# samxuxiang/BrepGen

Hardware: AMD Instinct MI355X
Metric: denoising-steps/sec (whole node), DeepCAD face-LDM, batch=512 (higher is better)
Workload: dtype bf16

## Files before the change

### brepgen_amd/csrc/qkv_attn.hip

```cpp
#include "gemm16.h"
#include <math.h>

namespace bg {

constexpr int QA_BUF = 57344, QA_AHALF = 16384, QA_WOFF = 32768, QA_RING = 2 * QA_BUF;
constexpr int QA_LDS = 163840;
constexpr int QA_AUX = QA_RING, QA_BIAS = QA_LDS - QA_AUX - 2048, QA_CSUM = QA_BIAS + 1024;
constexpr int QA_QIMG = QA_BUF, QA_KIMG = QA_QIMG + 32768, QA_VIMG = QA_KIMG + 32768;

constexpr int QA_MB = QA_AUX + QA_BIAS - 1024;
static_assert(QA_VIMG + 32768 <= QA_MB && QA_VIMG + 32768 <= QA_AUX + QA_BIAS, "the V image ends below the key bias / bias / column sums");

struct QkvAttnArgs {
    const void* a;
    const void* w;
    const float* bias;
    const float* colsum;
    const float* stats_in;
    void* out;
    void* dbg;
    const uint8_t* key_pad;
    int B, N, M;
    float ln_eps;
    const int* m_dev = nullptr;
    const int* slot_desc = nullptr;
    int pin = 0;
};

typedef __attribute__((ext_vector_type(4))) short qa_v4s;

__device__ __forceinline__ int qa_opaque(int x) {
    asm volatile("" : "+v"(x));
    return x;
}

template <bool F16, int S, bool MASK, bool DBG = false, bool PAIR = false>
__global__ __launch_bounds__(512) void qkv_attn_kernel(QkvAttnArgs g) {
    using E = Elem<F16>;
    using T = typename E::T;
    using V8 = typename E::V8;
    using V4 = typename E::V4;
    constexpr int SPT = 256 / S;
    constexpr int WPS = S / 32;
    constexpr int LD = BG_D_MODEL;
    __shared__ __attribute__((aligned(16))) unsigned char lds[QA_LDS];

    const int wave = __builtin_amdgcn_readfirstlane(threadIdx.x >> 6);
    const int wm = wave >> 1, wn = (wave ^ (wave >> 2)) & 1;
    const int late = wave >> 2;
    static_assert(!PAIR || (S == 64 && !MASK), "slot-packed batches: 64-row slots, dead keys come from the slot descriptors");
    const int Mv = PAIR ? *g.m_dev : 0;
    const int n_groups = PAIR ? (Mv + 255) >> 8 : (g.B + SPT - 1) / SPT;
    const int T_all = n_groups * BG_N_HEAD;
    const int G = gridDim.x;
    int L = xcd_remap(blockIdx.x, G);
    const bool pin = g.pin != 0;
    const int pin_q = (blockIdx.x & 7) >> 1, pin_h0 = (blockIdx.x & 1) * 6, pin_step = G >> 3;
    auto tile_of = [&](int l, int& tg, int& th) -> bool {
        if (pin) { tg = 4 * (l / 6) + pin_q; th = pin_h0 + l % 6; return tg < n_groups; }
        tg = l / BG_N_HEAD; th = l % BG_N_HEAD;
        return l < T_all;
    };
    if (pin) L = blockIdx.x >> 3;
    {
        int tg, th;
        if (!tile_of(L, tg, th)) return;
    }

    const unsigned char* Ab = reinterpret_cast<const unsigned char*>(g.a);
    const unsigned char* Wb = reinterpret_cast<const unsigned char*>(g.w);
    constexpr unsigned lda_b = LD * 2u, ldw_b = LD * 2u;
    const unsigned lds0 = __builtin_amdgcn_readfirstlane((unsigned)(size_t)(__attribute__((address_space(3))) void*)lds);
    const unsigned aux_lds = lds0 + QA_AUX;
    const unsigned char* aux = lds + QA_AUX;

    auto dma = [&](unsigned dst, const unsigned char* src, unsigned voff) {
        unsigned keep;
        asm volatile("s_mov_b32 %0, m0\n\ts_mov_b32 m0, %3\n\ts_nop 0\n\tglobal_load_lds_dwordx4 %1, %2\n\ts_mov_b32 m0, %0"
                     : "=&s"(keep) : "v"(voff), "s"(src), "s"(dst) : "memory");
    };

    auto bar = [&]() {
        asm volatile("" ::: "memory");
        __builtin_amdgcn_sched_barrier(0);
        __builtin_amdgcn_s_barrier();
        __builtin_amdgcn_sched_barrier(0);
        asm volatile("" ::: "memory");
    };
    auto lds_done_bar = [&]() {
        asm volatile("s_waitcnt lgkmcnt(0)" ::: "memory");
        bar();
    };

    unsigned ha[2][2], hw;
    auto piece_row = [&](int ln, int r) { return (wave + 8 * r) * 8 + (ln >> 3); };
    auto piece_chunk = [&](int ln, int r) { return (unsigned)(((ln & 7) ^ ((piece_row(ln, r) >> 1) & 7)) * 16); };
    auto slot_row = [&](int grp, int tile_row) {
        if (PAIR) {
            const int row = grp * 256 + tile_row;
            return row < Mv ? row : Mv - 1;
        }
        int smp = grp * SPT + tile_row / S;
        smp = smp < g.B ? smp : g.B - 1;
        int tok = tile_row % S;
        tok = tok < g.N ? tok : g.N - 1;
        return smp * g.N + tok;
    };
    auto a_offsets = [&](int grp) {
        const int ln = qa_opaque(threadIdx.x & 63);
#pragma unroll
        for (int hh = 0; hh < 2; ++hh)
#pragma unroll
            for (int r = 0; r < 2; ++r)
                ha[hh][r] = (unsigned)slot_row(grp, hh * 128 + piece_row(ln, r)) * lda_b + piece_chunk(ln, r);
    };
    {
        const int ln = threadIdx.x & 63;
        hw = (unsigned)piece_row(ln, 0) * ldw_b + piece_chunk(ln, 0);
    }
    auto stage_a = [&](int buf, const unsigned char* src) {
#pragma unroll
        for (int hh = 0; hh < 2; ++hh)
#pragma unroll
            for (int r = 0; r < 2; ++r)
                dma(lds0 + (unsigned)(buf * QA_BUF + hh * QA_AHALF + (wave + 8 * r) * 1024), src, ha[hh][r]);
    };
    auto stage_w = [&](int buf, const unsigned char* src) {
#pragma unroll
        for (int c3 = 0; c3 < 3; ++c3)
            dma(lds0 + (unsigned)(buf * QA_BUF + QA_WOFF + (wave + 8 * c3) * 1024), src + (size_t)c3 * LD * ldw_b, hw);
    };
    auto stage_stats = [&](int grp) {
        const int ln = qa_opaque(threadIdx.x & 63);
        const int gh = wave >> 2;
        int row = slot_row(grp, gh * 128 + 2 * ln);
        row = (row & 1) ? row - 1 : row;
        const unsigned char* sb = reinterpret_cast<const unsigned char*>(g.stats_in);
#pragma unroll
        for (int r = 0; r < 3; ++r) {
            const int part = (wave & 3) * 3 + r;
            dma(aux_lds + (unsigned)(gh * 12288 + part * 1024), sb + (size_t)part * (size_t)g.M * 8, (unsigned)(row >> 1) * 16u);
        }
    };
    auto stage_cols = [&](int head) {
        const int ln = qa_opaque(threadIdx.x & 63);
        int c3 = ln >> 4;
        c3 = c3 < 3 ? c3 : 2;
        const unsigned voff = (unsigned)(c3 * LD + (ln & 15) * 4) * 4u;
        if (wave == 0) dma(aux_lds + QA_BIAS, reinterpret_cast<const unsigned char*>(g.bias + head * 64), voff);
        if (wave == 1) dma(aux_lds + QA_CSUM, reinterpret_cast<const unsigned char*>(g.colsum + head * 64), voff);
    };

    unsigned a_rd, b_rd, xk[4];
    {
        const int ln = threadIdx.x & 63, l31 = ln & 31, hq = ln >> 5, sw = (l31 >> 1) & 7;
        a_rd = (unsigned)(wm * 64 + l31) * 128u;
        b_rd = (unsigned)QA_WOFF + (unsigned)(wn * 96 + l31) * 128u;
#pragma unroll
        for (int ks = 0; ks < 4; ++ks) xk[ks] = (unsigned)(((ks * 2 + hq) ^ sw) << 4);
    }
    f32x16 acc[2][3];
    V8 fa[2][4], fb[3][4];
    auto read_a = [&](const unsigned char* st) {
#pragma unroll
        for (int i = 0; i < 2; ++i)
#pragma unroll
            for (int ks = 0; ks < 4; ++ks) fa[i][ks] = *reinterpret_cast<const V8*>(st + a_rd + i * 4096 + xk[ks]);
    };
    auto read_b = [&](const unsigned char* st, int j) {
#pragma unroll
        for (int ks = 0; ks < 4; ++ks) fb[j][ks] = *reinterpret_cast<const V8*>(st + b_rd + j * 4096 + xk[ks]);
    };
    auto segment = [&](int j) {
        asm volatile("s_waitcnt lgkmcnt(0)" ::: "memory");
        __builtin_amdgcn_sched_barrier(0);
        __builtin_amdgcn_s_setprio(1);
#pragma unroll
        for (int ks = 0; ks < 4; ++ks)
#pragma unroll
            for (int i = 0; i < 2; ++i) acc[i][j] = E::mfma(fb[j][ks], fa[i][ks], acc[i][j]);
        __builtin_amdgcn_s_setprio(0);
        __builtin_amdgcn_sched_barrier(0);
    };

    constexpr int KT = LD / G_BK;
    const unsigned char* b0 = lds;
    const unsigned char* b1 = lds + QA_BUF;

    int grp, head;
    tile_of(L, grp, head);
    float2 cf[2];
    auto fold_sums = [&](int i) {
        const int l31 = qa_opaque(threadIdx.x & 31);
        const unsigned char* sg = aux + (wm >> 1) * 12288;
        const int rg = (wm & 1) * 64 + i * 32 + l31;
        float ps[16], pq[16];
#pragma unroll
        for (int pp = 0; pp < 16; ++pp) {
            const float2 v = pp < FOLD_PARTS ? reinterpret_cast<const float2*>(sg + pp * 1024)[rg] : make_float2(0.f, 0.f);
            ps[pp] = v.x; pq[pp] = v.y;
        }
        cf[i] = make_float2(tree16(ps), tree16(pq));
        asm volatile("" : "+v"(cf[i].x), "+v"(cf[i].y) :: "memory");
        __builtin_amdgcn_sched_barrier(0);
    };
    auto fold_coeffs = [&](int i) {
        cf[i] = ln_fold_coeffs(cf[i].x, cf[i].y, LD, g.ln_eps);
        asm volatile("" : "+v"(cf[i].x), "+v"(cf[i].y) :: "memory");
        __builtin_amdgcn_sched_barrier(0);
    };

    a_offsets(grp);
    stage_stats(grp); stage_cols(head);
    stage_a(0, Ab); stage_w(0, Wb + (size_t)head * 64 * ldw_b); stage_a(1, Ab + 2 * G_BK);
    wait_vmcnt<4>();
    bar();
    for (;;) {
        if (late) bar();
        const unsigned char* w_cur = Wb + (size_t)head * 64 * ldw_b;
        const int Ln = L + (pin ? pin_step : G);
        int grp_n, head_n;
        const bool has_next = tile_of(Ln, grp_n, head_n);
        const unsigned char* w_nxt = Wb + (size_t)head_n * 64 * ldw_b;
#pragma unroll
        for (int i = 0; i < 2; ++i)
#pragma unroll
            for (int j = 0; j < 3; ++j)
#pragma unroll
                for (int r = 0; r < 16; ++r) acc[i][j][r] = 0.f;

        auto iteration = [&](const unsigned char* w1, bool more, const unsigned char* a2, const unsigned char* w2, bool more3,
                             const unsigned char* a3, int fold) {
            read_b(b0, 0); __builtin_amdgcn_sched_barrier(0); read_a(b0);
            stage_w(1, w1);
            bar(); segment(0); bar();
            read_b(b0, 1); read_b(b0, 2);
            bar(); segment(1); bar();
            if (more) { stage_a(0, a2); wait_vmcnt<4>(); } else { wait_vmcnt<0>(); }
            if (fold >= 0) fold_sums(fold);
            bar(); segment(2); bar();
            read_b(b1, 0); __builtin_amdgcn_sched_barrier(0); read_a(b1);
            if (more) stage_w(0, w2);
            bar(); segment(0); bar();
            read_b(b1, 1); read_b(b1, 2);
            bar(); segment(1); bar();
            if (more3) { stage_a(1, a3); wait_vmcnt<4>(); } else if (more) { wait_vmcnt<0>(); }
            if (fold >= 0) fold_coeffs(fold);
            bar(); segment(2); bar();
        };
        for (int t = 0; t + 2 < KT; t += 2) {
            const unsigned kb = (unsigned)t * (2 * G_BK);
            iteration(w_cur + kb + 2 * G_BK, true, Ab + kb + 4 * G_BK, w_cur + kb + 4 * G_BK, true, Ab + kb + 6 * G_BK,
                      t == KT - 6 ? 0 : (t == KT - 4 ? 1 : -1));
        }
        if (has_next) a_offsets(grp_n);
        iteration(w_cur + (unsigned)(KT - 1) * (2 * G_BK), has_next, Ab, w_nxt, false, Ab, -1);
        if (!late) bar();

        const int ln = qa_opaque(threadIdx.x & 63), l31 = ln & 31, hq = ln >> 5;
        T* dbg = reinterpret_cast<T*>(g.dbg);
        int pair_na = 64, pair_nb = 0;
        if (PAIR) {
            const int gslot = grp * 4 + wm;
            if (gslot * 64 < Mv) { pair_na = g.slot_desc[2 * gslot]; pair_nb = g.slot_desc[2 * gslot + 1]; }
            pair_na = __builtin_amdgcn_readfirstlane(pair_na);
            pair_nb = __builtin_amdgcn_readfirstlane(pair_nb);
        }
        float key_bias = 0.f;
        if (MASK && threadIdx.x < 256) {
            const int smp = grp * SPT + (int)threadIdx.x / S, key = (int)threadIdx.x % S;
            const bool inside = smp < g.B && key < g.N;
            const uint8_t pad = inside ? g.key_pad[(size_t)smp * g.N + key] : (uint8_t)1;
            key_bias = pad ? -INFINITY : 0.f;
        }
#pragma unroll
        for (int j = 0; j < 3; ++j) {
            const int tc0 = wn * 96 + j * 32;
            const int c3 = tc0 >> 6, d0 = tc0 & 63;
#pragma unroll
            for (int q = 0; q < 4; ++q) {
                const int d = d0 + 8 * q + 4 * hq;
                const float4 bz = *reinterpret_cast<const float4*>(aux + QA_BIAS + (unsigned)(c3 * 64 + d) * 4u);
                const float4 cs = *reinterpret_cast<const float4*>(aux + QA_CSUM + (unsigned)(c3 * 64 + d) * 4u);
                const float b4[4] = {bz.x, bz.y, bz.z, bz.w}, c4[4] = {cs.x, cs.y, cs.z, cs.w};
#pragma unroll
                for (int i = 0; i < 2; ++i) {
                    float v[4];
#pragma unroll
                    for (int e = 0; e < 4; ++e) v[e] = ln_fold_apply(acc[i][j][4 * q + e], cf[i].x, cf[i].y, c4[e], b4[e]);
                    if (F16) asm volatile("" : "+v"(v[0]), "+v"(v[1]), "+v"(v[2]), "+v"(v[3]));
                    union { V4 v; uint2 u; T t[4]; } pk;
                    pk.v = E::pack4(v[0], v[1], v[2], v[3]);
                    const int R = wm * 64 + i * 32 + l31;
                    *reinterpret_cast<uint2*>(lds + QA_QIMG + c3 * 32768 + R * 128 + ((((d >> 3) ^ ((R >> 1) & 7))) << 4) + (d & 7) * 2) = pk.u;
                    if (DBG) {
                        const int smp = grp * SPT + R / S, tok = R % S;
                        if (PAIR ? grp * 256 + R < Mv : (smp < g.B && tok < g.N))
                            *reinterpret_cast<uint2*>(dbg + (size_t)(PAIR ? grp * 256 + R : smp * g.N + tok) * (3 * LD) + c3 * LD + head * 64 + d) = pk.u;
                    }
                }
            }
        }
        if (MASK && threadIdx.x < 256) reinterpret_cast<float*>(lds + QA_MB)[threadIdx.x] = key_bias;
        lds_done_bar();

        if (has_next) stage_cols(head_n);

        {
            const int wq = wm * 2 + wn;
            const int slot = wq / WPS, qb = wq % WPS;
            const int smp = grp * SPT + slot;
            if (PAIR ? (grp * 256 + slot * 64 < Mv) : (smp < g.B)) {
                const int h = hq;
                const unsigned char* qimg = lds + QA_QIMG + (slot * S + qb * 32) * 128;
                const unsigned char* ktile = lds + QA_KIMG + slot * S * 128;
                const unsigned char* vimg = lds + QA_VIMG + slot * S * 128;
                const int gi = ln & 15, gg = ln >> 4;
                const int v_key0 = 4 * (gg >> 1) + (gi >> 2);
                int v_c16[2], v_b8;
                v_b8 = ((gi & 3) * 4 & 7) * 2;
#pragma unroll
                for (int dt = 0; dt < 2; ++dt) v_c16[dt] = (dt * 32 + (gg & 1) * 16 + (gi & 3) * 4) >> 3;
                const int sw = (l31 >> 1) & 7;
                V8 qf[4];
#pragma unroll
                for (int ks = 0; ks < 4; ++ks) qf[ks] = *reinterpret_cast<const V8*>(qimg + l31 * 128 + (((ks * 2 + h) ^ sw) << 4));
                f32x16 o[2];
#pragma unroll
                for (int dt = 0; dt < 2; ++dt)
#pragma unroll
                    for (int r = 0; r < 16; ++r) o[dt][r] = 0.f;
                float m_run = -INFINITY, l_run = 0.f;
                const int tq = qb * 32 + l31;
                const bool in_b = PAIR && tq >= pair_na && tq < pair_na + pair_nb;
                bool first = true;
#pragma unroll
                for (int si = 0; si < (PAIR ? 2 : 1); ++si) {
                    const int cnt = PAIR ? (si == 0 ? pair_na : pair_nb) : g.N;
                    const int row0 = (PAIR && si == 1) ? pair_na : 0;
                    const bool member = !PAIR || (in_b == (si == 1));
                    if (PAIR && __ballot(member) == 0ull) continue;
#pragma unroll
                    for (int sub = 0; sub < WPS; ++sub) {
                        if (sub * 32 >= cnt) break;
                        f32x16 s;
#pragma unroll
                        for (int r = 0; r < 16; ++r) s[r] = 0.f;
                        int kr = row0 + sub * 32 + l31;
                        if (PAIR) kr = kr < 63 ? kr : 63;
                        const int ksw = PAIR ? (kr >> 1) & 7 : sw;
#pragma unroll
                        for (int ks = 0; ks < 4; ++ks) {
                            const V8 kf = *reinterpret_cast<const V8*>(ktile + kr * 128 + (((ks * 2 + h) ^ ksw) << 4));
                            s = E::mfma(kf, qf[ks], s);
                        }
                        if (MASK) {
                            const float* mb = reinterpret_cast<const float*>(lds + QA_MB) + slot * S + sub * 32 + 4 * h;
#pragma unroll
                            for (int g4 = 0; g4 < 4; ++g4) {
                                const float4 mbv = *reinterpret_cast<const float4*>(mb + 8 * g4);
                                s[4 * g4 + 0] += mbv.x; s[4 * g4 + 1] += mbv.y; s[4 * g4 + 2] += mbv.z; s[4 * g4 + 3] += mbv.w;
                            }
                        } else if (PAIR) {
                            const int thr = member ? cnt - sub * 32 - 4 * h : -64;
#pragma unroll
                            for (int r = 0; r < 16; ++r) s[r] += ((r & 3) + 8 * (r >> 2)) >= thr ? -INFINITY : 0.f;
                        } else if (sub * 32 + 32 > g.N) {
                            const int thr = g.N - sub * 32 - 4 * h;
#pragma unroll
                            for (int r = 0; r < 16; ++r) s[r] += ((r & 3) + 8 * (r >> 2)) >= thr ? -INFINITY : 0.f;
                        }
                        float mloc = -INFINITY;
#pragma unroll
                        for (int g4 = 0; g4 < 4; ++g4)
                            mloc = fmaxf(mloc, fmaxf(fmaxf(s[4 * g4 + 0], s[4 * g4 + 1]), fmaxf(s[4 * g4 + 2], s[4 * g4 + 3])));
                        mloc = fmaxf(mloc, __shfl_xor(mloc, 32, 64));
                        const float m_new = fmaxf(m_run, mloc);
                        const float m_use = (m_new == -INFINITY) ? 0.f : m_new;
                        float psum = 0.f;
#pragma unroll
                        for (int r = 0; r < 16; ++r) {
                            s[r] = __expf(s[r] - m_use);
                            psum += s[r];
                        }
                        if (first) {
                            l_run = psum;
                        } else {
                            const float alpha = __expf(m_run - m_use);
                            l_run = l_run * alpha + psum;
#pragma unroll
                            for (int dt = 0; dt < 2; ++dt)
#pragma unroll
                                for (int r = 0; r < 16; ++r) o[dt][r] *= alpha;
                        }
                        first = false;
                        m_run = m_new;
#pragma unroll
                        for (int sl = 0; sl < 2; ++sl) {
                            V8 pb;
#pragma unroll
                            for (int e = 0; e < 8; ++e) pb[e] = (T)s[8 * sl + e];
                            int r_lo = row0 + sub * 32 + 16 * sl + v_key0, r_hi = r_lo + 8;
                            if (PAIR) { r_lo = r_lo < 63 ? r_lo : 63; r_hi = r_hi < 63 ? r_hi : 63; }
#pragma unroll
                            for (int dt = 0; dt < 2; ++dt) {
                                const unsigned char* pl = vimg + r_lo * 128 + ((v_c16[dt] ^ ((r_lo >> 1) & 7)) << 4) + v_b8;
                                const unsigned char* ph = vimg + r_hi * 128 + ((v_c16[dt] ^ ((r_hi >> 1) & 7)) << 4) + v_b8;
                                union { qa_v4s s4[2]; V8 v; } vau;
                                vau.s4[0] = __builtin_amdgcn_ds_read_tr16_b64_v4i16((__attribute__((address_space(3))) qa_v4s*)pl);
                                vau.s4[1] = __builtin_amdgcn_ds_read_tr16_b64_v4i16((__attribute__((address_space(3))) qa_v4s*)ph);
                                const V8 va = vau.v;
                                o[dt] = E::mfma(va, pb, o[dt]);
                            }
                        }
                    }
                }
                const float l_tot = l_run + __shfl_xor(l_run, 32, 64);
                const float inv = l_tot > 0.f ? 1.0f / l_tot : 0.f;
                if (PAIR || tq < g.N) {
                    T* op = reinterpret_cast<T*>(g.out) + (size_t)(PAIR ? grp * 256 + slot * 64 + tq : smp * g.N + tq) * LD + head * 64;
#pragma unroll
                    for (int dt = 0; dt < 2; ++dt)
#pragma unroll
                        for (int k2 = 0; k2 < 2; ++k2) {
                            union { V4 v; unsigned u[2]; } q0, q1;
                            q0.v[0] = cvt16<T>(o[dt][8 * k2 + 0] * inv); q0.v[1] = cvt16<T>(o[dt][8 * k2 + 1] * inv);
                            q0.v[2] = cvt16<T>(o[dt][8 * k2 + 2] * inv); q0.v[3] = cvt16<T>(o[dt][8 * k2 + 3] * inv);
                            q1.v[0] = cvt16<T>(o[dt][8 * k2 + 4] * inv); q1.v[1] = cvt16<T>(o[dt][8 * k2 + 5] * inv);
                            q1.v[2] = cvt16<T>(o[dt][8 * k2 + 6] * inv); q1.v[3] = cvt16<T>(o[dt][8 * k2 + 7] * inv);
                            const auto w0 = __builtin_amdgcn_permlane32_swap(q0.u[0], q1.u[0], false, false);
                            const auto w1 = __builtin_amdgcn_permlane32_swap(q0.u[1], q1.u[1], false, false);
                            const uint4 st16 = make_uint4(w0[0], w1[0], w0[1], w1[1]);
                            *reinterpret_cast<uint4*>(op + dt * 32 + 16 * k2 + 8 * h) = st16;
                        }
                }
            }
        }
        if (!has_next) break;
        lds_done_bar();
        L = Ln; grp = grp_n; head = head_n;
        stage_a(1, Ab + 2 * G_BK);
        stage_stats(grp);
    }
}

bool qkv_attn_eligible(int B, int N, int dtype, const void* stats_in, const void* colsum, const void* bias) {
    return (dtype == BG_BF16 || dtype == BG_F16) && B > 0 && N >= 2 && N <= 64 && (N & 1) == 0 && stats_in && colsum && bias &&
           (((size_t)stats_in) & 15) == 0 && (size_t)B * N * BG_D_MODEL * 2 < 0xffffffffull;
}

bool qkv_attn_worthwhile(int B, int N) {
    const int spt = N <= 32 ? 8 : 4;
    const int tiles = (B + spt - 1) / spt * BG_N_HEAD;
    return tiles <= 256 || tiles >= 352;
}

static int qkv_attn_pinned_walk(int tiles, int grid) {
    const int t = g_tune[TUNE_QKV_WALK];
    if (t == 1 || (grid & 7) != 0) return 0;
    return (t == 2 || tiles >= 512) ? 1 : 0;
}

int qkv_attention_launch(const QkvAttnArgs& g, int dtype, hipStream_t s) {
    const int S = g.N <= 32 ? 32 : 64, spt = 256 / S;
    const int tiles = (g.B + spt - 1) / spt * BG_N_HEAD;
    if (tiles <= 0) return 0;
    const double rows = (double)g.B * g.N;
    ProfScope prof(PK_QKV_ATTN, 2.0 * rows * BG_D_MODEL * 3 * BG_D_MODEL + 4.0 * BG_N_HEAD * (double)g.B * g.N * g.N * BG_D_HEAD,
                   rows * (2.0 * BG_D_MODEL * 2 + FOLD_PARTS * 8.0) + 2.0 * 3 * BG_D_MODEL * BG_D_MODEL + 2 * 4.0 * 3 * BG_D_MODEL, s);
    const int grid = tiles < 256 ? tiles : 256;
    const bool f16 = dtype == BG_F16;
    QkvAttnArgs ge = g;
    ge.pin = qkv_attn_pinned_walk(tiles, grid);
#define QA_LAUNCH(F, SS, MK, D) hipLaunchKernelGGL((qkv_attn_kernel<F, SS, MK, D>), dim3(grid), dim3(512), 0, s, ge)
#define QA_PICK(MK, D)                                                                                     \
    do {                                                                                                   \
        if (S == 64) { if (f16) QA_LAUNCH(true, 64, MK, D); else QA_LAUNCH(false, 64, MK, D); }           \
        else { if (f16) QA_LAUNCH(true, 32, MK, D); else QA_LAUNCH(false, 32, MK, D); }                   \
    } while (0)
    if (g.dbg) {
        if (g.key_pad) QA_PICK(true, true); else QA_PICK(false, true);
    } else {
        if (g.key_pad) QA_PICK(true, false); else QA_PICK(false, false);
    }
#undef QA_PICK
#undef QA_LAUNCH
    return launch_status("qkv_attn");
}

int qkv_attention_paired(const void* x_hi, const void* w_qkv, const float* bias, const float* colsum, const float* stats_in, void* out,
                         void* qkv_dbg, const int* m_dev, const int* slot_desc, int slot_bound, int m_stats, int dtype, float ln_eps,
                         hipStream_t s, double rows_hint, double pairs_hint) {
    if (slot_bound <= 0) return 0;
    QkvAttnArgs g{x_hi, w_qkv, bias, colsum, stats_in, out, qkv_dbg, nullptr, slot_bound, 64, m_stats, ln_eps};
    g.m_dev = m_dev;
    g.slot_desc = slot_desc;
    const int tiles = (slot_bound + 3) / 4 * BG_N_HEAD;
    g.pin = qkv_attn_pinned_walk(tiles, tiles < 256 ? tiles : 256);
    const double rows = rows_hint > 0 ? rows_hint : 64.0 * slot_bound;
    const double pairs = pairs_hint > 0 ? pairs_hint : 64.0 * rows;
    ProfScope prof(PK_QKV_ATTN, 2.0 * rows * BG_D_MODEL * 3 * BG_D_MODEL + 4.0 * BG_N_HEAD * pairs * BG_D_HEAD,
                   rows * (2.0 * BG_D_MODEL * 2 + FOLD_PARTS * 8.0) + 2.0 * 3 * BG_D_MODEL * BG_D_MODEL + 2 * 4.0 * 3 * BG_D_MODEL, s);
    const int grid = tiles < 256 ? tiles : 256;
    if (dtype == BG_F16) {
        if (qkv_dbg) hipLaunchKernelGGL((qkv_attn_kernel<true, 64, false, true, true>), dim3(grid), dim3(512), 0, s, g);
        else hipLaunchKernelGGL((qkv_attn_kernel<true, 64, false, false, true>), dim3(grid), dim3(512), 0, s, g);
    } else {
        if (qkv_dbg) hipLaunchKernelGGL((qkv_attn_kernel<false, 64, false, true, true>), dim3(grid), dim3(512), 0, s, g);
        else hipLaunchKernelGGL((qkv_attn_kernel<false, 64, false, false, true>), dim3(grid), dim3(512), 0, s, g);
    }
    return launch_status("qkv_attn_paired");
}

int qkv_attention(const void* x_hi, const void* w_qkv, const float* bias, const float* colsum, const float* stats_in, void* out,
                  const uint8_t* key_pad, int B, int N, int dtype, float ln_eps, hipStream_t s) {
    const QkvAttnArgs g{x_hi, w_qkv, bias, colsum, stats_in, out, nullptr, key_pad, B, N, B * N, ln_eps};
    return qkv_attention_launch(g, dtype, s);
}

}

extern "C" int bg_qkv_attn_fwd(const void* x_hi, const void* w_qkv, const float* bias, const float* colsum, const float* stats_in,
                               const uint8_t* key_pad, void* out, void* qkv_dbg, int B, int N, int dtype, float ln_eps,
                               bg_stream_t stream) {
    BG_REQUIRE(x_hi && w_qkv && out && B >= 0 && N >= 0, BG_E_ARG, "bg_qkv_attn_fwd: null pointer or negative size");
    BG_REQUIRE(bg::qkv_attn_eligible(B, N, dtype, stats_in, colsum, bias), BG_E_SHAPE,
               "bg_qkv_attn_fwd: needs 16-bit operands, an even N in [2, 64], LayerNorm-fold statistics / column sums / bias (16-byte aligned)");
    BG_REQUIRE(((uintptr_t)x_hi & 15) == 0 && ((uintptr_t)w_qkv & 15) == 0 && ((uintptr_t)out & 15) == 0 &&
               ((uintptr_t)bias & 15) == 0 && ((uintptr_t)colsum & 15) == 0, BG_E_ALIGN, "bg_qkv_attn_fwd: 16-byte alignment");
    bg::QkvAttnArgs g{x_hi, w_qkv, bias, colsum, stats_in, out, qkv_dbg, key_pad, B, N, B * N, ln_eps};
    return bg::qkv_attention_launch(g, dtype, (hipStream_t)stream);
}

extern "C" int bg_qkv_attn_paired_fwd(const void* x_hi, const void* w_qkv, const float* bias, const float* colsum, const float* stats_in,
                                      void* out, void* qkv_dbg, const int* m_dev, const int* slot_desc, int slot_bound, int m_stats,
                                      int dtype, float ln_eps, bg_stream_t stream) {
    BG_REQUIRE(x_hi && w_qkv && out && m_dev && slot_desc && slot_bound > 0 && m_stats >= 64 * slot_bound, BG_E_ARG,
               "bg_qkv_attn_paired_fwd: null pointer, or a statistics stride below 64 rows per slot");
    BG_REQUIRE((dtype == BG_BF16 || dtype == BG_F16) && stats_in && colsum && bias && (m_stats & 1) == 0, BG_E_SHAPE,
               "bg_qkv_attn_paired_fwd: 16-bit operands with LayerNorm-fold statistics / column sums / bias");
    BG_REQUIRE(((uintptr_t)x_hi & 15) == 0 && ((uintptr_t)w_qkv & 15) == 0 && ((uintptr_t)out & 15) == 0 && ((uintptr_t)bias & 15) == 0 &&
               ((uintptr_t)colsum & 15) == 0 && ((uintptr_t)stats_in & 15) == 0, BG_E_ALIGN, "bg_qkv_attn_paired_fwd: 16-byte alignment");
    BG_REQUIRE((size_t)64 * slot_bound * BG_D_MODEL * 2 < 0xffffffffull, BG_E_SHAPE, "bg_qkv_attn_paired_fwd: more than 43 690 slots");
    return bg::qkv_attention_paired(x_hi, w_qkv, bias, colsum, stats_in, out, qkv_dbg, m_dev, slot_desc, slot_bound, m_stats, dtype, ln_eps,
                                    (hipStream_t)stream, 0.0, 0.0);
}
```

Before: 370.5.

## Replace block barrier with pairwise wave flags and batch attention LDS loads

In the unmasked path, the block-wide barrier between writing the Q/K/V images and the attention phase becomes a pairwise handshake through LDS flags, so each wave waits only on its partner wave. The attention inner loop now loads all K and V fragments for a sample up front before issuing the MFMAs. The loop is templated on sub-tile count, and the cross-half shuffles use permlane32_swap instead of __shfl_xor. Bias and column-sum loads are hoisted into registers, and stage_cols moves after the end-of-tile barrier. The risks are higher register pressure and the correctness of the flag protocol, which assumes only the partner wave's image rows are read. Optional timestamp probes are added behind a macro.

```diff
diff --git a/brepgen_amd/csrc/qkv_attn.hip b/brepgen_amd/csrc/qkv_attn.hip
--- a/brepgen_amd/csrc/qkv_attn.hip
+++ b/brepgen_amd/csrc/qkv_attn.hip
@@ -1,5 +1,6 @@
 #include "gemm16.h"
 #include <math.h>
+#include <type_traits>
 
 namespace bg {
 
@@ -10,6 +11,8 @@
 
 constexpr int QA_MB = QA_AUX + QA_BIAS - 1024;
 static_assert(QA_VIMG + 32768 <= QA_MB && QA_VIMG + 32768 <= QA_AUX + QA_BIAS, "the V image ends below the key bias / bias / column sums");
+constexpr int QA_FLAG = QA_VIMG + 32768;
+static_assert(QA_FLAG + 32 <= QA_MB, "the image flags end below the key bias");
 
 struct QkvAttnArgs {
     const void* a;
@@ -25,7 +28,21 @@
     const int* m_dev = nullptr;
     const int* slot_desc = nullptr;
     int pin = 0;
+#ifdef QA_STAMPS
+    long long* stamps = nullptr;
+#endif
 };
+
+#ifdef QA_STAMPS
+constexpr int QA_STAMP_TILES = 16;
+#define QA_STAMP(k)                                                                                                              \
+    do {                                                                                                                         \
+        if (g.stamps && blockIdx.x == 0 && (threadIdx.x & 255) == 0 && n_tile < QA_STAMP_TILES)                                 \
+            g.stamps[((threadIdx.x >> 8) * QA_STAMP_TILES + n_tile) * 8 + (k)] = (long long)__builtin_amdgcn_s_memtime();      \
+    } while (0)
+#else
+#define QA_STAMP(k) do {} while (0)
+#endif
 
 typedef __attribute__((ext_vector_type(4))) short qa_v4s;
 
@@ -213,10 +230,17 @@
     a_offsets(grp);
     stage_stats(grp); stage_cols(head);
     stage_a(0, Ab); stage_w(0, Wb + (size_t)head * 64 * ldw_b); stage_a(1, Ab + 2 * G_BK);
+    volatile __attribute__((address_space(3))) int* img_flag = (volatile __attribute__((address_space(3))) int*)(lds + QA_FLAG);
+    if ((threadIdx.x & 63) == 0) img_flag[wave] = 0;
+    int img_seq = 0;
     wait_vmcnt<4>();
     bar();
+#ifdef QA_STAMPS
+    int n_tile = 0;
+#endif
     for (;;) {
         if (late) bar();
+        QA_STAMP(0);
         const unsigned char* w_cur = Wb + (size_t)head * 64 * ldw_b;
         const int Ln = L + (pin ? pin_step : G);
         int grp_n, head_n;
@@ -256,6 +280,7 @@
         if (has_next) a_offsets(grp_n);
         iteration(w_cur + (unsigned)(KT - 1) * (2 * G_BK), has_next, Ab, w_nxt, false, Ab, -1);
         if (!late) bar();
+        QA_STAMP(1);
 
         const int ln = qa_opaque(threadIdx.x & 63), l31 = ln & 31, hq = ln >> 5;
         T* dbg = reinterpret_cast<T*>(g.dbg);
@@ -273,6 +298,15 @@
             const uint8_t pad = inside ? g.key_pad[(size_t)smp * g.N + key] : (uint8_t)1;
             key_bias = pad ? -INFINITY : 0.f;
         }
+        float4 bzq[3][4], csq[3][4];
+#pragma unroll
+        for (int j = 0; j < 3; ++j)
+#pragma unroll
+            for (int q = 0; q < 4; ++q) {
+                const unsigned col = (unsigned)(wn * 96 + j * 32 + 8 * q + 4 * hq);
+                bzq[j][q] = *reinterpret_cast<const float4*>(aux + QA_BIAS + col * 4u);
+                csq[j][q] = *reinterpret_cast<const float4*>(aux + QA_CSUM + col * 4u);
+            }
 #pragma unroll
         for (int j = 0; j < 3; ++j) {
             const int tc0 = wn * 96 + j * 32;
@@ -280,8 +314,7 @@
 #pragma unroll
             for (int q = 0; q < 4; ++q) {
                 const int d = d0 + 8 * q + 4 * hq;
-                const float4 bz = *reinterpret_cast<const float4*>(aux + QA_BIAS + (unsigned)(c3 * 64 + d) * 4u);
-                const float4 cs = *reinterpret_cast<const float4*>(aux + QA_CSUM + (unsigned)(c3 * 64 + d) * 4u);
+                const float4 bz = bzq[j][q], cs = csq[j][q];
                 const float b4[4] = {bz.x, bz.y, bz.z, bz.w}, c4[4] = {cs.x, cs.y, cs.z, cs.w};
 #pragma unroll
                 for (int i = 0; i < 2; ++i) {
@@ -301,10 +334,19 @@
                 }
             }
         }
-        if (MASK && threadIdx.x < 256) reinterpret_cast<float*>(lds + QA_MB)[threadIdx.x] = key_bias;
-        lds_done_bar();
-
-        if (has_next) stage_cols(head_n);
+        QA_STAMP(2);
+        if (MASK) {
+            if (threadIdx.x < 256) reinterpret_cast<float*>(lds + QA_MB)[threadIdx.x] = key_bias;
+            lds_done_bar();
+        } else {
+            ++img_seq;
+            asm volatile("s_waitcnt lgkmcnt(0)" ::: "memory");
+            if (ln == 0) img_flag[wave] = img_seq;
+            while (__builtin_amdgcn_readfirstlane(img_flag[wave ^ 1]) != img_seq) __builtin_amdgcn_s_sleep(1);
+            asm volatile("" ::: "memory");
+            __builtin_amdgcn_sched_barrier(0);
+        }
+        QA_STAMP(3);
 
         {
             const int wq = wm * 2 + wn;
@@ -334,26 +376,49 @@
                 const int tq = qb * 32 + l31;
                 const bool in_b = PAIR && tq >= pair_na && tq < pair_na + pair_nb;
                 bool first = true;
-#pragma unroll
-                for (int si = 0; si < (PAIR ? 2 : 1); ++si) {
-                    const int cnt = PAIR ? (si == 0 ? pair_na : pair_nb) : g.N;
-                    const int row0 = (PAIR && si == 1) ? pair_na : 0;
-                    const bool member = !PAIR || (in_b == (si == 1));
-                    if (PAIR && __ballot(member) == 0ull) continue;
-#pragma unroll
-                    for (int sub = 0; sub < WPS; ++sub) {
-                        if (sub * 32 >= cnt) break;
-                        f32x16 s;
-#pragma unroll
-                        for (int r = 0; r < 16; ++r) s[r] = 0.f;
+                auto other_half = [&](float x) {
+                    const auto p2 = __builtin_amdgcn_permlane32_swap(__float_as_uint(x), __float_as_uint(x), false, false);
+                    return __uint_as_float(h ? p2[0] : p2[1]);
+                };
+                auto sample = [&](auto ns_tag, int cnt, int row0, bool member) {
+                    constexpr int NS = decltype(ns_tag)::value;
+                    V8 kf[NS][4], va[NS][2][2];
+#pragma unroll
+                    for (int sub = 0; sub < NS; ++sub) {
                         int kr = row0 + sub * 32 + l31;
                         if (PAIR) kr = kr < 63 ? kr : 63;
                         const int ksw = PAIR ? (kr >> 1) & 7 : sw;
 #pragma unroll
-                        for (int ks = 0; ks < 4; ++ks) {
-                            const V8 kf = *reinterpret_cast<const V8*>(ktile + kr * 128 + (((ks * 2 + h) ^ ksw) << 4));
-                            s = E::mfma(kf, qf[ks], s);
+                        for (int ks = 0; ks < 4; ++ks) kf[sub][ks] = *reinterpret_cast<const V8*>(ktile + kr * 128 + (((ks * 2 + h) ^ ksw) << 4));
+                    }
+#pragma unroll
+                    for (int sub = 0; sub < NS; ++sub)
+#pragma unroll
+                        for (int sl = 0; sl < 2; ++sl) {
+                            int r_lo = row0 + sub * 32 + 16 * sl + v_key0, r_hi = r_lo + 8;
+                            if (PAIR) { r_lo = r_lo < 63 ? r_lo : 63; r_hi = r_hi < 63 ? r_hi : 63; }
+#pragma unroll
+                            for (int dt = 0; dt < 2; ++dt) {
+                                const unsigned char* pl = vimg + r_lo * 128 + ((v_c16[dt] ^ ((r_lo >> 1) & 7)) << 4) + v_b8;
+                                const unsigned char* ph = vimg + r_hi * 128 + ((v_c16[dt] ^ ((r_hi >> 1) & 7)) << 4) + v_b8;
+                                union { qa_v4s s4[2]; V8 v; } vau;
+                                vau.s4[0] = __builtin_amdgcn_ds_read_tr16_b64_v4i16((__attribute__((address_space(3))) qa_v4s*)pl);
+                                vau.s4[1] = __builtin_amdgcn_ds_read_tr16_b64_v4i16((__attribute__((address_space(3))) qa_v4s*)ph);
+                                va[sub][sl][dt] = vau.v;
+                            }
                         }
+                    f32x16 sc[NS];
+#pragma unroll
+                    for (int sub = 0; sub < NS; ++sub)
+#pragma unroll
+                        for (int r = 0; r < 16; ++r) sc[sub][r] = 0.f;
+#pragma unroll
+                    for (int ks = 0; ks < 4; ++ks)
+#pragma unroll
+                        for (int sub = 0; sub < NS; ++sub) sc[sub] = E::mfma(kf[sub][ks], qf[ks], sc[sub]);
+#pragma unroll
+                    for (int sub = 0; sub < NS; ++sub) {
+                        f32x16& s = sc[sub];
                         if (MASK) {
                             const float* mb = reinterpret_cast<const float*>(lds + QA_MB) + slot * S + sub * 32 + 4 * h;
 #pragma unroll
@@ -374,7 +439,7 @@
 #pragma unroll
                         for (int g4 = 0; g4 < 4; ++g4)
                             mloc = fmaxf(mloc, fmaxf(fmaxf(s[4 * g4 + 0], s[4 * g4 + 1]), fmaxf(s[4 * g4 + 2], s[4 * g4 + 3])));
-                        mloc = fmaxf(mloc, __shfl_xor(mloc, 32, 64));
+                        mloc = fmaxf(mloc, other_half(mloc));
                         const float m_new = fmaxf(m_run, mloc);
                         const float m_use = (m_new == -INFINITY) ? 0.f : m_new;
                         float psum = 0.f;
@@ -400,22 +465,21 @@
                             V8 pb;
 #pragma unroll
                             for (int e = 0; e < 8; ++e) pb[e] = (T)s[8 * sl + e];
-                            int r_lo = row0 + sub * 32 + 16 * sl + v_key0, r_hi = r_lo + 8;
-                            if (PAIR) { r_lo = r_lo < 63 ? r_lo : 63; r_hi = r_hi < 63 ? r_hi : 63; }
-#pragma unroll
-                            for (int dt = 0; dt < 2; ++dt) {
-                                const unsigned char* pl = vimg + r_lo * 128 + ((v_c16[dt] ^ ((r_lo >> 1) & 7)) << 4) + v_b8;
-                                const unsigned char* ph = vimg + r_hi * 128 + ((v_c16[dt] ^ ((r_hi >> 1) & 7)) << 4) + v_b8;
-                                union { qa_v4s s4[2]; V8 v; } vau;
-                                vau.s4[0] = __builtin_amdgcn_ds_read_tr16_b64_v4i16((__attribute__((address_space(3))) qa_v4s*)pl);
-                                vau.s4[1] = __builtin_amdgcn_ds_read_tr16_b64_v4i16((__attribute__((address_space(3))) qa_v4s*)ph);
-                                const V8 va = vau.v;
-                                o[dt] = E::mfma(va, pb, o[dt]);
-                            }
+#pragma unroll
+                            for (int dt = 0; dt < 2; ++dt) o[dt] = E::mfma(va[sub][sl][dt], pb, o[dt]);
                         }
                     }
+                };
+#pragma unroll
+                for (int si = 0; si < (PAIR ? 2 : 1); ++si) {
+                    const int cnt = PAIR ? (si == 0 ? pair_na : pair_nb) : g.N;
+                    const int row0 = (PAIR && si == 1) ? pair_na : 0;
+                    const bool member = !PAIR || (in_b == (si == 1));
+                    if (PAIR && __ballot(member) == 0ull) continue;
+                    if (!PAIR || cnt > 32) sample(std::integral_constant<int, WPS>(), cnt, row0, member);
+                    else if (cnt > 0) sample(std::integral_constant<int, 1>(), cnt, row0, member);
                 }
-                const float l_tot = l_run + __shfl_xor(l_run, 32, 64);
+                const float l_tot = l_run + other_half(l_run);
                 const float inv = l_tot > 0.f ? 1.0f / l_tot : 0.f;
                 if (PAIR || tq < g.N) {
                     T* op = reinterpret_cast<T*>(g.out) + (size_t)(PAIR ? grp * 256 + slot * 64 + tq : smp * g.N + tq) * LD + head * 64;
@@ -436,9 +500,15 @@
                 }
             }
         }
+        QA_STAMP(4);
         if (!has_next) break;
         lds_done_bar();
+        QA_STAMP(5);
+#ifdef QA_STAMPS
+        ++n_tile;
+#endif
         L = Ln; grp = grp_n; head = head_n;
+        stage_cols(head);
         stage_a(1, Ab + 2 * G_BK);
         stage_stats(grp);
     }
```

New measurement: 372.6, median of 6. Within noise of the previous version (+0.6%).
